# jackroos/VL-BERT

Hardware: AMD Instinct MI355X
Metric: samples/sec VL-BERT-base pretrain (seq 64+36 regions) at 1/2/4/8 MI355X (higher is better)
Workload: dtype bf16; 1 GPU; VL-BERT-base 12-layer pretrain step (fwd+bwd+clip+AdamW), 64 text + 36 regions, precomputed 2048-d region features, dropout on; global_batch=256, per_gpu_batch=256, per_gpu_caption_samples=256, per_gpu_text_only_samples=0, module=ResNetVLBERTForPretraining, seq_len=101, parallelism=dp1, hipgraph=False, arch=gfx950:sramecc+:xnack-, cus=256, forced_exchange=False, ranks=1

## Files before the change

vl-bert_amd/csrc/attention.hip:

```cpp
#include "vlb_common.h"

#define ATT_SP_MAX 256
#define ATT_D 64
#define ATT_THREADS 512

typedef __attribute__((ext_vector_type(4))) short s16x4;
typedef __attribute__((ext_vector_type(8))) short s16x8;

__device__ __forceinline__ int rho(int s) { return (s & ~31) | (((s >> 2) & 1) << 4) | (((s >> 3) & 3) << 2) | (s & 3); }
__device__ __forceinline__ int rm_addr(int row, int chunk) { return row * 128 + ((chunk ^ ((row >> 1) & 7)) << 4); }
__device__ __forceinline__ bf16x8 lds_frag(const char* base, int addr) { return *(const bf16x8*)(base + addr); }

__device__ __forceinline__ bf16x8 frag_perm(const char* img, int blk, int half, int c, int chunk) {
  return lds_frag(img, rm_addr(32 * blk + 16 * half + c, chunk));
}
__device__ __forceinline__ bf16x8 frag_nat(const char* img, int s0, int c, int chunk) {
  return lds_frag(img, rm_addr(rho(s0 + c), chunk));
}
__device__ __forceinline__ bf16x8 frag_tr(const char* img, int blk, int d0, int lane) {
  const int L = lane & 15, g = lane >> 4;
  const int b = d0 * 2 + (L & 3) * 8;
  const int r_lo = 32 * blk + 4 * g + (L >> 2);
  const int r_hi = r_lo + 16;
  const int a_lo = r_lo * 128 + ((((b >> 4) ^ ((r_lo >> 1) & 7)) << 4) | (b & 15));
  const int a_hi = r_hi * 128 + ((((b >> 4) ^ ((r_hi >> 1) & 7)) << 4) | (b & 15));
  const s16x4 lo = __builtin_amdgcn_ds_read_tr16_b64_v4i16((__attribute__((address_space(3))) s16x4*)(img + a_lo));
  const s16x4 hi = __builtin_amdgcn_ds_read_tr16_b64_v4i16((__attribute__((address_space(3))) s16x4*)(img + a_hi));
  const s16x8 v = __builtin_shufflevector(lo, hi, 0, 1, 2, 3, 4, 5, 6, 7);
  return __builtin_bit_cast(bf16x8, v);
}

template <int SP>
struct TileRegs {
  uint4 v[SP * 8 / ATT_THREADS];
};

template <int SP>
__device__ __forceinline__ void tile_load(const bf16_t* __restrict__ g, long ld, int S, int tid, TileRegs<SP>& r) {
#pragma unroll
  for (int it = 0; it < SP * 8 / ATT_THREADS; ++it) {
    const int P = it * ATT_THREADS + tid, s = min(P >> 3, S - 1), ch = P & 7;
    r.v[it] = *(const uint4*)(g + (long)s * ld + ch * 8);
  }
}

template <int SP>
__device__ __forceinline__ void tile_store(const TileRegs<SP>& r, int S, char* img, int tid) {
#pragma unroll
  for (int it = 0; it < SP * 8 / ATT_THREADS; ++it) {
    const int P = it * ATT_THREADS + tid, s = P >> 3, ch = P & 7;
    const bool in = s < S;
    const uint4 v = make_uint4(in ? r.v[it].x : 0u, in ? r.v[it].y : 0u, in ? r.v[it].z : 0u, in ? r.v[it].w : 0u);
    *(uint4*)(img + rm_addr(rho(s), ch)) = v;
  }
}

template <int SP>
__device__ __forceinline__ void rowdot_store(const TileRegs<SP>& a_, const TileRegs<SP>& o_, int S, float* sD, int tid) {
#pragma unroll
  for (int it = 0; it < SP * 8 / ATT_THREADS; ++it) {
    const int P = it * ATT_THREADS + tid, row = P >> 3, ch = P & 7;
    const uint4 a = a_.v[it], o = o_.v[it];
    float d = bflo(a.x) * bflo(o.x) + bfhi(a.x) * bfhi(o.x) + bflo(a.y) * bflo(o.y) + bfhi(a.y) * bfhi(o.y) +
              bflo(a.z) * bflo(o.z) + bfhi(a.z) * bfhi(o.z) + bflo(a.w) * bflo(o.w) + bfhi(a.w) * bfhi(o.w);
    d = row < S ? d : 0.f;
    d += __shfl_xor(d, 1, 64);
    d += __shfl_xor(d, 2, 64);
    d += __shfl_xor(d, 4, 64);
    if (ch == 0) sD[row] = d;
  }
}

__device__ __forceinline__ bf16x8 pack8(const float* v) {
  uint32_t w[4] = {pack2bf(v[0], v[1]), pack2bf(v[2], v[3]), pack2bf(v[4], v[5]), pack2bf(v[6], v[7])};
  return __builtin_bit_cast(bf16x8, *(uint4*)w);
}

__device__ __forceinline__ void drop8(float* v, uint32_t key, uint32_t base, uint32_t thr, float scale) {
  const uint32_t odd = base & 1u, p0 = base >> 1;
  uint32_t h[5];
#pragma unroll
  for (int k = 0; k < 5; ++k) h[k] = vlb_pair_hash(p0 + k, key);
#pragma unroll
  for (int k = 0; k < 4; ++k) {
    const uint32_t w = __builtin_amdgcn_alignbit(h[k + 1], h[k], odd << 4);
    v[2 * k] = ((w & 0xffffu) >= thr) ? v[2 * k] * scale : 0.f;
    v[2 * k + 1] = ((w >> 16) >= thr) ? v[2 * k + 1] * scale : 0.f;
  }
}

struct AttnParams {
  const bf16_t* qkv;
  const float* mask;
  bf16_t* ctx;
  float* lse;
  const bf16_t* dctx;
  bf16_t* dqkv;
  int B, S, H, nh;
  float scale;
  uint32_t drop_thr; float drop_scale; const uint32_t* seed; uint32_t tag;
};

template <int NU, int QS>
__global__ __launch_bounds__(ATT_THREADS, NU <= 4 ? 4 : 2) void attn_fwd_kernel(const AttnParams p) {
  constexpr int ATT_SP = 32 * NU, TILE_BYTES = ATT_SP * ATT_D * 2;
  extern __shared__ __attribute__((aligned(16))) char smem[];
  char* sK = smem;
  char* sV = smem + TILE_BYTES;
  float* sMB = (float*)(smem + 2 * TILE_BYTES);

  const int tid = threadIdx.x, lane = tid & 63, wave = tid >> 6;
  const int c = lane & 15, g = lane >> 4;
  const int b = blockIdx.x / p.nh, h = blockIdx.x % p.nh;
  const int S = p.S;
  const long ld = 3L * p.H;
  const bf16_t* qbase = p.qkv + (long)b * S * ld + h * ATT_D;
  TileRegs<ATT_SP> rk, rv;
  tile_load<ATT_SP>(qbase + p.H, ld, S, tid, rk);
  tile_load<ATT_SP>(qbase + 2 * p.H, ld, S, tid, rv);
  bf16x8 qf[2];
  auto load_q = [&](int q0) {
    const int q = min(q0 + c, S - 1);
#pragma unroll
    for (int ds = 0; ds < 2; ++ds) qf[ds] = *(const bf16x8*)(qbase + (long)q * ld + ds * 32 + g * 8);
  };
  load_q(wave * 16);
  const float mrow = p.mask[b * S + min(tid, S - 1)];
  const uint32_t seed = (p.drop_thr && p.seed) ? *p.seed : 0u;
  tile_store<ATT_SP>(rk, S, sK, tid);
  tile_store<ATT_SP>(rv, S, sV, tid);
  if (tid < ATT_SP) sMB[tid] = (tid < S) ? (1.0f - mrow) * -10000.0f : -INFINITY;
  __syncthreads();
  const uint32_t key = vlb_rng_key(seed, p.tag);
  const int U = (S + 31) >> 5;

#pragma unroll 1
  for (int qs = 0; qs < QS; ++qs) {
  const int q0 = (wave + 8 * qs) * 16;
  if (q0 >= S) break;
  if (qs > 0) load_q(q0);

  f32x4 sc[NU][2];
#pragma unroll
  for (int u = 0; u < NU; ++u)
#pragma unroll
    for (int hf = 0; hf < 2; ++hf) {
      sc[u][hf] = (f32x4){0.f, 0.f, 0.f, 0.f};
      if (u < U) {
#pragma unroll
        for (int ds = 0; ds < 2; ++ds)
          sc[u][hf] = VLB_MFMA_16x16x32(frag_perm(sK, u, hf, c, ds * 4 + g), qf[ds], sc[u][hf], 0, 0, 0);
      }
    }

  float mx = -INFINITY;
#pragma unroll
  for (int u = 0; u < NU; ++u)
#pragma unroll
    for (int hf = 0; hf < 2; ++hf)
#pragma unroll
      for (int r = 0; r < 4; ++r) {
        const float v = (u < U) ? sc[u][hf][r] * p.scale + sMB[32 * u + 8 * g + 4 * hf + r] : -INFINITY;
        sc[u][hf][r] = v;
        mx = fmaxf(mx, v);
      }
  mx = fmaxf(mx, __shfl_xor(mx, 16, 64));
  mx = fmaxf(mx, __shfl_xor(mx, 32, 64));
  float sum = 0.f;
#pragma unroll
  for (int u = 0; u < NU; ++u)
#pragma unroll
    for (int hf = 0; hf < 2; ++hf)
#pragma unroll
      for (int r = 0; r < 4; ++r) {
        const float e = __expf(sc[u][hf][r] - mx);
        sc[u][hf][r] = e;
        sum += e;
      }
  sum += __shfl_xor(sum, 16, 64);
  sum += __shfl_xor(sum, 32, 64);
  const float inv = 1.0f / sum;
  const int q = q0 + c;
  if (g == 0 && q < S) p.lse[((long)b * p.nh + h) * S + q] = mx + __logf(sum);

  const uint32_t qrow = ((uint32_t)(b * p.nh + h) * (uint32_t)S + (uint32_t)min(q, S - 1)) * (uint32_t)S;
  bf16x8 pf[NU];
#pragma unroll
  for (int u = 0; u < NU; ++u) {
    float v[8];
#pragma unroll
    for (int hf = 0; hf < 2; ++hf)
#pragma unroll
      for (int r = 0; r < 4; ++r) v[4 * hf + r] = sc[u][hf][r] * inv;
    if (p.drop_thr) drop8(v, key, qrow + 32u * u + 8u * g, p.drop_thr, p.drop_scale);
    pf[u] = pack8(v);
  }

  bf16_t* orow = p.ctx + ((long)b * S + min(q, S - 1)) * p.H + h * ATT_D + 4 * g;
#pragma unroll
  for (int dt = 0; dt < 4; ++dt) {
    f32x4 o = {0.f, 0.f, 0.f, 0.f};
#pragma unroll
    for (int u = 0; u < NU; ++u)
      if (u < U) o = VLB_MFMA_16x16x32(frag_tr(sV, u, dt * 16, lane), pf[u], o, 0, 0, 0);
    if (q < S) *(uint2*)(orow + dt * 16) = make_uint2(pack2bf(o[0], o[1]), pack2bf(o[2], o[3]));
  }
  }
}

template <int NU, int QS>
__global__ __launch_bounds__(ATT_THREADS, NU <= 4 ? 4 : 2) void attn_bwd_kernel(const AttnParams p) {
  constexpr int ATT_SP = 32 * NU, TILE_BYTES = ATT_SP * ATT_D * 2;
  extern __shared__ __attribute__((aligned(16))) char smem[];
  char* sQ = smem;
  char* sK = smem + 1 * TILE_BYTES;
  char* sV = smem + 2 * TILE_BYTES;
  char* sdO = smem + 3 * TILE_BYTES;
  float* sMB = (float*)(smem + 4 * TILE_BYTES);
  float* sLSE = sMB + ATT_SP;
  float* sD = sLSE + ATT_SP;

  const int tid = threadIdx.x, lane = tid & 63, wave = tid >> 6;
  const int c = lane & 15, g = lane >> 4;
  const int b = blockIdx.x / p.nh, h = blockIdx.x % p.nh;
  const int S = p.S;
  const long ld = 3L * p.H;
  const bf16_t* qbase = p.qkv + (long)b * S * ld + h * ATT_D;
  const bf16_t* dobase = p.dctx + (long)b * S * p.H + h * ATT_D;
  const bf16_t* obase = p.ctx + (long)b * S * p.H + h * ATT_D;
  TileRegs<ATT_SP> rq, rk, rv, rdo, ro;
  tile_load<ATT_SP>(qbase, ld, S, tid, rq);
  tile_load<ATT_SP>(qbase + p.H, ld, S, tid, rk);
  tile_load<ATT_SP>(qbase + 2 * p.H, ld, S, tid, rv);
  tile_load<ATT_SP>(dobase, p.H, S, tid, rdo);
  tile_load<ATT_SP>(obase, p.H, S, tid, ro);
  const float mrow = p.mask[b * S + min(tid, S - 1)];
  const float lrow = p.lse[((long)b * p.nh + h) * S + min(tid, S - 1)];
  const uint32_t seed = (p.drop_thr && p.seed) ? *p.seed : 0u;
  tile_store<ATT_SP>(rq, S, sQ, tid);
  tile_store<ATT_SP>(rk, S, sK, tid);
  tile_store<ATT_SP>(rv, S, sV, tid);
  tile_store<ATT_SP>(rdo, S, sdO, tid);
  rowdot_store<ATT_SP>(rdo, ro, S, sD, tid);
  if (tid < ATT_SP) {
    sMB[tid] = (tid < S) ? (1.0f - mrow) * -10000.0f : -INFINITY;
    sLSE[tid] = (tid < S) ? lrow : 0.f;
  }
  __syncthreads();

  const uint32_t key = vlb_rng_key(seed, p.tag);
  const uint32_t bh = (uint32_t)(b * p.nh + h);
  const int U = (S + 31) >> 5;
#pragma unroll 1
  for (int qs = 0; qs < QS; ++qs) {
  const int w16 = (wave + 8 * qs) * 16;
  if (w16 >= S) break;
  const int pos = w16 + c;
  const bool pos_ok = pos < S;

  {
    bf16x8 kf[2], vf[2];
#pragma unroll
    for (int ds = 0; ds < 2; ++ds) {
      kf[ds] = frag_nat(sK, w16, c, ds * 4 + g);
      vf[ds] = frag_nat(sV, w16, c, ds * 4 + g);
    }
    f32x4 dv[4], dk[4];
#pragma unroll
    for (int dt = 0; dt < 4; ++dt) dv[dt] = dk[dt] = (f32x4){0.f, 0.f, 0.f, 0.f};
    const float mb = sMB[pos];
    const uint32_t kcol = (uint32_t)min(pos, S - 1);
#pragma unroll (NU <= 4 ? NU : 1)
    for (int v = 0; v < NU; ++v) {
      if (v < U) {
        float pv[8], dsv[8];
#pragma unroll
        for (int hf = 0; hf < 2; ++hf) {
          f32x4 s = {0.f, 0.f, 0.f, 0.f}, dp = {0.f, 0.f, 0.f, 0.f};
#pragma unroll
          for (int ds = 0; ds < 2; ++ds) {
            s = VLB_MFMA_16x16x32(frag_perm(sQ, v, hf, c, ds * 4 + g), kf[ds], s, 0, 0, 0);
            dp = VLB_MFMA_16x16x32(frag_perm(sdO, v, hf, c, ds * 4 + g), vf[ds], dp, 0, 0, 0);
          }
#pragma unroll
          for (int r = 0; r < 4; ++r) {
            const int q = 32 * v + 8 * g + 4 * hf + r;
            const float pr = __expf(s[r] * p.scale + mb - sLSE[q]);
            float keepf = 1.f;
            if (p.drop_thr) {
              const uint32_t idx = (bh * (uint32_t)S + (uint32_t)min(q, S - 1)) * (uint32_t)S + kcol;
              const uint32_t hsh = vlb_pair_hash(idx >> 1, key);
              keepf = (((idx & 1u) ? (hsh >> 16) : (hsh & 0xffffu)) >= p.drop_thr) ? p.drop_scale : 0.f;
            }
            pv[4 * hf + r] = pr * keepf;
            dsv[4 * hf + r] = pr * (dp[r] * keepf - sD[q]);
          }
        }
        const bf16x8 pd = pack8(pv), dsf = pack8(dsv);
#pragma unroll
        for (int dt = 0; dt < 4; ++dt) {
          dv[dt] = VLB_MFMA_16x16x32(frag_tr(sdO, v, dt * 16, lane), pd, dv[dt], 0, 0, 0);
          dk[dt] = VLB_MFMA_16x16x32(frag_tr(sQ, v, dt * 16, lane), dsf, dk[dt], 0, 0, 0);
        }
      }
    }
    if (pos_ok) {
      bf16_t* orow = p.dqkv + ((long)b * S + pos) * ld + h * ATT_D + 4 * g;
#pragma unroll
      for (int dt = 0; dt < 4; ++dt) {
        *(uint2*)(orow + p.H + dt * 16) = make_uint2(pack2bf(dk[dt][0] * p.scale, dk[dt][1] * p.scale),
                                                     pack2bf(dk[dt][2] * p.scale, dk[dt][3] * p.scale));
        *(uint2*)(orow + 2 * p.H + dt * 16) = make_uint2(pack2bf(dv[dt][0], dv[dt][1]), pack2bf(dv[dt][2], dv[dt][3]));
      }
    }
  }

  {
    bf16x8 qf[2], dof[2];
#pragma unroll
    for (int ds = 0; ds < 2; ++ds) {
      qf[ds] = frag_nat(sQ, w16, c, ds * 4 + g);
      dof[ds] = frag_nat(sdO, w16, c, ds * 4 + g);
    }
    f32x4 dq[4];
#pragma unroll
    for (int dt = 0; dt < 4; ++dt) dq[dt] = (f32x4){0.f, 0.f, 0.f, 0.f};
    const float lse = sLSE[pos], dd = sD[pos];
    const uint32_t qrow = (bh * (uint32_t)S + (uint32_t)min(pos, S - 1)) * (uint32_t)S;
#pragma unroll (NU <= 4 ? NU : 1)
    for (int u = 0; u < NU; ++u) {
      if (u < U) {
        float pr[8], dpv[8];
#pragma unroll
        for (int hf = 0; hf < 2; ++hf) {
          f32x4 s = {0.f, 0.f, 0.f, 0.f}, dp = {0.f, 0.f, 0.f, 0.f};
#pragma unroll
          for (int ds = 0; ds < 2; ++ds) {
            s = VLB_MFMA_16x16x32(frag_perm(sK, u, hf, c, ds * 4 + g), qf[ds], s, 0, 0, 0);
            dp = VLB_MFMA_16x16x32(frag_perm(sV, u, hf, c, ds * 4 + g), dof[ds], dp, 0, 0, 0);
          }
#pragma unroll
          for (int r = 0; r < 4; ++r) {
            pr[4 * hf + r] = __expf(s[r] * p.scale + sMB[32 * u + 8 * g + 4 * hf + r] - lse);
            dpv[4 * hf + r] = dp[r];
          }
        }
        if (p.drop_thr) drop8(dpv, key, qrow + 32u * u + 8u * g, p.drop_thr, p.drop_scale);
        float dsv[8];
#pragma unroll
        for (int j = 0; j < 8; ++j) dsv[j] = pr[j] * (dpv[j] - dd);
        const bf16x8 dsf = pack8(dsv);
#pragma unroll
        for (int dt = 0; dt < 4; ++dt)
          dq[dt] = VLB_MFMA_16x16x32(frag_tr(sK, u, dt * 16, lane), dsf, dq[dt], 0, 0, 0);
      }
    }
    if (pos_ok) {
      bf16_t* orow = p.dqkv + ((long)b * S + pos) * ld + h * ATT_D + 4 * g;
#pragma unroll
      for (int dt = 0; dt < 4; ++dt)
        *(uint2*)(orow + dt * 16) = make_uint2(pack2bf(dq[dt][0] * p.scale, dq[dt][1] * p.scale),
                                               pack2bf(dq[dt][2] * p.scale, dq[dt][3] * p.scale));
    }
  }
  }
}

__device__ __forceinline__ int pt_addr(int row, int chunk16) { return row * 256 + ((chunk16 ^ (row & 15)) << 4); }

__device__ __forceinline__ bf16x8 frag_pt(const char* img, int v, int key0, int lane) {
  const int L = lane & 15, g = lane >> 4;
  const int r_lo = 32 * v + 8 * g + (L >> 2), r_hi = r_lo + 4;
  const int cb = key0 * 2 + (L & 3) * 8;
  const int a_lo = pt_addr(r_lo, cb >> 4) | (cb & 15), a_hi = pt_addr(r_hi, cb >> 4) | (cb & 15);
  const s16x4 lo = __builtin_amdgcn_ds_read_tr16_b64_v4i16((__attribute__((address_space(3))) s16x4*)(img + a_lo));
  const s16x4 hi = __builtin_amdgcn_ds_read_tr16_b64_v4i16((__attribute__((address_space(3))) s16x4*)(img + a_hi));
  const s16x8 w = __builtin_shufflevector(lo, hi, 0, 1, 2, 3, 4, 5, 6, 7);
  return __builtin_bit_cast(bf16x8, w);
}

__global__ __launch_bounds__(ATT_THREADS, 4) void attn_bwd2_kernel(const AttnParams p) {
  constexpr int NU = 4, ATT_SP = 128, TILE_BYTES = ATT_SP * ATT_D * 2;
  extern __shared__ __attribute__((aligned(16))) char smem[];
  char* sQ = smem;
  char* sK = smem + 1 * TILE_BYTES;
  char* sV = smem + 2 * TILE_BYTES;
  char* sdO = smem + 3 * TILE_BYTES;
  char* sT = sK;
  float* sMB = (float*)(smem + 4 * TILE_BYTES);
  float* sLSE = sMB + ATT_SP;
  float* sD = sLSE + ATT_SP;

  const int tid = threadIdx.x, lane = tid & 63, wave = tid >> 6;
  const int c = lane & 15, g = lane >> 4;
  const int b = blockIdx.x / p.nh, h = blockIdx.x % p.nh;
  const int S = p.S;
  const long ld = 3L * p.H;
  const bf16_t* qbase = p.qkv + (long)b * S * ld + h * ATT_D;
  const bf16_t* dobase = p.dctx + (long)b * S * p.H + h * ATT_D;
  const bf16_t* obase = p.ctx + (long)b * S * p.H + h * ATT_D;
  TileRegs<ATT_SP> rq, rk, rv, rdo, ro;
  tile_load<ATT_SP>(qbase, ld, S, tid, rq);
  tile_load<ATT_SP>(qbase + p.H, ld, S, tid, rk);
  tile_load<ATT_SP>(qbase + 2 * p.H, ld, S, tid, rv);
  tile_load<ATT_SP>(dobase, p.H, S, tid, rdo);
  tile_load<ATT_SP>(obase, p.H, S, tid, ro);
  const float mrow = p.mask[b * S + min(tid, S - 1)];
  const float lrow = p.lse[((long)b * p.nh + h) * S + min(tid, S - 1)];
  const uint32_t seed = (p.drop_thr && p.seed) ? *p.seed : 0u;
  tile_store<ATT_SP>(rq, S, sQ, tid);
  tile_store<ATT_SP>(rk, S, sK, tid);
  tile_store<ATT_SP>(rv, S, sV, tid);
  tile_store<ATT_SP>(rdo, S, sdO, tid);
  rowdot_store<ATT_SP>(rdo, ro, S, sD, tid);
  if (tid < ATT_SP) {
    sMB[tid] = (tid < S) ? (1.0f - mrow) * -10000.0f : -INFINITY;
    sLSE[tid] = (tid < S) ? lrow : 0.f;
  }
  __syncthreads();

  const uint32_t key = vlb_rng_key(seed, p.tag);
  const uint32_t bh = (uint32_t)(b * p.nh + h);
  const int U = (S + 31) >> 5;
  const int w16 = wave * 16;
  const int pos = w16 + c;
  const bool pos_ok = pos < S;
  const bool active = w16 < 32 * U;

  bf16x8 pd[NU], dsf[NU];
#pragma unroll
  for (int u = 0; u < NU; ++u) pd[u] = dsf[u] = (bf16x8){0, 0, 0, 0, 0, 0, 0, 0};
  if (w16 < S) {
    bf16x8 qf[2], dof[2];
#pragma unroll
    for (int ds = 0; ds < 2; ++ds) {
      qf[ds] = frag_nat(sQ, w16, c, ds * 4 + g);
      dof[ds] = frag_nat(sdO, w16, c, ds * 4 + g);
    }
    f32x4 dq[4];
#pragma unroll
    for (int dt = 0; dt < 4; ++dt) dq[dt] = (f32x4){0.f, 0.f, 0.f, 0.f};
    const float lse = sLSE[pos], dd = sD[pos];
    const float rowf = pos_ok ? 1.f : 0.f;
    const uint32_t qrow = (bh * (uint32_t)S + (uint32_t)min(pos, S - 1)) * (uint32_t)S;
#pragma unroll
    for (int u = 0; u < NU; ++u) {
      if (u < U) {
        float pr[8], dpv[8], kv[8];
#pragma unroll
        for (int hf = 0; hf < 2; ++hf) {
          f32x4 sc = {0.f, 0.f, 0.f, 0.f}, dp = {0.f, 0.f, 0.f, 0.f};
#pragma unroll
          for (int ds = 0; ds < 2; ++ds) {
            sc = VLB_MFMA_16x16x32(frag_perm(sK, u, hf, c, ds * 4 + g), qf[ds], sc, 0, 0, 0);
            dp = VLB_MFMA_16x16x32(frag_perm(sV, u, hf, c, ds * 4 + g), dof[ds], dp, 0, 0, 0);
          }
#pragma unroll
          for (int r = 0; r < 4; ++r) {
            pr[4 * hf + r] = __expf(sc[r] * p.scale + sMB[32 * u + 8 * g + 4 * hf + r] - lse) * rowf;
            dpv[4 * hf + r] = dp[r];
            kv[4 * hf + r] = 1.f;
          }
        }
        if (p.drop_thr) drop8(kv, key, qrow + 32u * u + 8u * g, p.drop_thr, p.drop_scale);
        float pdv[8], dsv[8];
#pragma unroll
        for (int j = 0; j < 8; ++j) {
          pdv[j] = pr[j] * kv[j];
          dsv[j] = pr[j] * (dpv[j] * kv[j] - dd);
        }
        pd[u] = pack8(pdv);
        dsf[u] = pack8(dsv);
#pragma unroll
        for (int dt = 0; dt < 4; ++dt)
          dq[dt] = VLB_MFMA_16x16x32(frag_tr(sK, u, dt * 16, lane), dsf[u], dq[dt], 0, 0, 0);
      }
    }
    if (pos_ok) {
      bf16_t* orow = p.dqkv + ((long)b * S + pos) * ld + h * ATT_D + 4 * g;
#pragma unroll
      for (int dt = 0; dt < 4; ++dt)
        *(uint2*)(orow + dt * 16) = make_uint2(pack2bf(dq[dt][0] * p.scale, dq[dt][1] * p.scale),
                                               pack2bf(dq[dt][2] * p.scale, dq[dt][3] * p.scale));
    }
  }
  __syncthreads();

  f32x4 dv[4], dk[4];
#pragma unroll
  for (int dt = 0; dt < 4; ++dt) dv[dt] = dk[dt] = (f32x4){0.f, 0.f, 0.f, 0.f};
  if (active) {
#pragma unroll
    for (int u = 0; u < NU; ++u)
      if (u < U) *(bf16x8*)(sT + pt_addr(w16 + c, 4 * u + g)) = pd[u];
  }
  __syncthreads();
  if (w16 < S) {
#pragma unroll
    for (int v = 0; v < NU; ++v) {
      if (v < U) {
        const bf16x8 pt = frag_pt(sT, v, w16, lane);
#pragma unroll
        for (int dt = 0; dt < 4; ++dt)
          dv[dt] = VLB_MFMA_16x16x32(frag_tr(sdO, v, dt * 16, lane), pt, dv[dt], 0, 0, 0);
      }
    }
  }
  __syncthreads();
  if (active) {
#pragma unroll
    for (int u = 0; u < NU; ++u)
      if (u < U) *(bf16x8*)(sT + pt_addr(w16 + c, 4 * u + g)) = dsf[u];
  }
  __syncthreads();
  if (w16 < S) {
#pragma unroll
    for (int v = 0; v < NU; ++v) {
      if (v < U) {
        const bf16x8 st = frag_pt(sT, v, w16, lane);
#pragma unroll
        for (int dt = 0; dt < 4; ++dt)
          dk[dt] = VLB_MFMA_16x16x32(frag_tr(sQ, v, dt * 16, lane), st, dk[dt], 0, 0, 0);
      }
    }
    if (pos_ok) {
      bf16_t* orow = p.dqkv + ((long)b * S + pos) * ld + h * ATT_D + 4 * g;
#pragma unroll
      for (int dt = 0; dt < 4; ++dt) {
        *(uint2*)(orow + p.H + dt * 16) = make_uint2(pack2bf(dk[dt][0] * p.scale, dk[dt][1] * p.scale),
                                                     pack2bf(dk[dt][2] * p.scale, dk[dt][3] * p.scale));
        *(uint2*)(orow + 2 * p.H + dt * 16) = make_uint2(pack2bf(dv[dt][0], dv[dt][1]), pack2bf(dv[dt][2], dv[dt][3]));
      }
    }
  }
}

static int check_attn(const char* name, int B, int S, int H, int nh) {
  VLB_CHECK_ARG(B > 0 && S > 0 && S <= ATT_SP_MAX, "%s: S=%d unsupported (1..%d)", name, S, ATT_SP_MAX);
  VLB_CHECK_ARG(nh > 0 && H == nh * ATT_D, "%s: head dim must be 64 (H=%d, heads=%d)", name, H, nh);
  VLB_CHECK_ARG((long)B * nh * S * S < (1L << 32), "%s: dropout index overflow", name);
  return VLB_OK;
}

extern "C" int vlb_attention_fwd(const void* qkv, const float* mask, void* ctx, float* lse, int B, int S, int H, int nh,
                                 float drop_p, const uint32_t* seed, uint32_t tag, hipStream_t stream) {
  int rc = check_attn("vlb_attention_fwd", B, S, H, nh);
  if (rc) return rc;
  VLB_CHECK_ARG(qkv && mask && ctx && lse, "vlb_attention_fwd: null argument");
  VLB_CHECK_ARG(!(drop_p > 0.f) || seed, "vlb_attention_fwd: dropout needs a device seed pointer");
  AttnParams p;
  p.qkv = (const bf16_t*)qkv; p.mask = mask; p.ctx = (bf16_t*)ctx; p.lse = lse; p.dctx = nullptr; p.dqkv = nullptr;
  p.B = B; p.S = S; p.H = H; p.nh = nh; p.scale = 0.125f;
  p.drop_thr = vlb_drop_thr(drop_p); p.drop_scale = vlb_drop_scale(p.drop_thr); p.seed = seed; p.tag = tag;
  if (S <= 128) {
    const int smem = 2 * (128 * ATT_D * 2) + 128 * 4;
    hipLaunchKernelGGL((attn_fwd_kernel<4, 1>), dim3(B * nh), dim3(ATT_THREADS), smem, stream, p);
  } else {
    const int smem = 2 * (256 * ATT_D * 2) + 256 * 4;
    static bool attr_set = false;
    if (!attr_set) {
      (void)hipFuncSetAttribute((const void*)attn_fwd_kernel<8, 2>, hipFuncAttributeMaxDynamicSharedMemorySize, smem);
      attr_set = true;
    }
    hipLaunchKernelGGL((attn_fwd_kernel<8, 2>), dim3(B * nh), dim3(ATT_THREADS), smem, stream, p);
  }
  VLB_CHECK_LAUNCH("vlb_attention_fwd");
  return VLB_OK;
}

extern "C" int vlb_attention_bwd(const void* qkv, const float* mask, const void* ctx, const float* lse, const void* dctx,
                                 void* dqkv, int B, int S, int H, int nh, float drop_p, const uint32_t* seed, uint32_t tag,
                                 hipStream_t stream) {
  int rc = check_attn("vlb_attention_bwd", B, S, H, nh);
  if (rc) return rc;
  VLB_CHECK_ARG(qkv && mask && ctx && lse && dctx && dqkv, "vlb_attention_bwd: null argument");
  VLB_CHECK_ARG(!(drop_p > 0.f) || seed, "vlb_attention_bwd: dropout needs a device seed pointer");
  AttnParams p;
  p.qkv = (const bf16_t*)qkv; p.mask = mask; p.ctx = (bf16_t*)ctx; p.lse = (float*)lse; p.dctx = (const bf16_t*)dctx;
  p.dqkv = (bf16_t*)dqkv;
  p.B = B; p.S = S; p.H = H; p.nh = nh; p.scale = 0.125f;
  p.drop_thr = vlb_drop_thr(drop_p); p.drop_scale = vlb_drop_scale(p.drop_thr); p.seed = seed; p.tag = tag;
  static bool attr_set = false;
  if (!attr_set) {
    (void)hipFuncSetAttribute((const void*)attn_bwd_kernel<4, 1>, hipFuncAttributeMaxDynamicSharedMemorySize, 4 * (128 * ATT_D * 2) + 3 * 128 * 4);
    (void)hipFuncSetAttribute((const void*)attn_bwd2_kernel, hipFuncAttributeMaxDynamicSharedMemorySize, 4 * (128 * ATT_D * 2) + 3 * 128 * 4);
    (void)hipFuncSetAttribute((const void*)attn_bwd_kernel<8, 2>, hipFuncAttributeMaxDynamicSharedMemorySize, 4 * (256 * ATT_D * 2) + 3 * 256 * 4);
    attr_set = true;
  }
  static int bwd2 = -1;
  if (bwd2 < 0) {
    const char* v = getenv("VLB_ATTN_BWD2");
    bwd2 = v ? atoi(v) : 1;
  }
  if (S <= 128 && bwd2)
    hipLaunchKernelGGL(attn_bwd2_kernel, dim3(B * nh), dim3(ATT_THREADS), 4 * (128 * ATT_D * 2) + 3 * 128 * 4, stream, p);
  else if (S <= 128)
    hipLaunchKernelGGL((attn_bwd_kernel<4, 1>), dim3(B * nh), dim3(ATT_THREADS), 4 * (128 * ATT_D * 2) + 3 * 128 * 4, stream, p);
  else
    hipLaunchKernelGGL((attn_bwd_kernel<8, 2>), dim3(B * nh), dim3(ATT_THREADS), 4 * (256 * ATT_D * 2) + 3 * 256 * 4, stream, p);
  VLB_CHECK_LAUNCH("vlb_attention_bwd");
  return VLB_OK;
}
```

Before: 13170 samples/s.

## Stage attention backward dQ/dK/dV through LDS for coalesced row stores

In attn_bwd2_kernel, the dQ, dK and dV outputs are written into a per-wave LDS staging area (reusing the dO tile region) and then flushed as full 16-byte row chunks. This replaces the scattered 8-byte strided global stores. The LDS swizzle keys for the row-major and transposed tiles are also changed, to cut bank conflicts on the read_tr and staging accesses. The change adds wave-level fences plus extra LDS traffic, and it depends on sdO no longer being read when the staging writes happen.

```diff
diff --git a/vl-bert_amd/csrc/attention.hip b/vl-bert_amd/csrc/attention.hip
--- a/vl-bert_amd/csrc/attention.hip
+++ b/vl-bert_amd/csrc/attention.hip
@@ -8,7 +8,8 @@
 typedef __attribute__((ext_vector_type(8))) short s16x8;
 
 __device__ __forceinline__ int rho(int s) { return (s & ~31) | (((s >> 2) & 1) << 4) | (((s >> 3) & 3) << 2) | (s & 3); }
-__device__ __forceinline__ int rm_addr(int row, int chunk) { return row * 128 + ((chunk ^ ((row >> 1) & 7)) << 4); }
+__device__ __forceinline__ int rm_key(int row) { return ((row >> 1) & 3) << 1; }
+__device__ __forceinline__ int rm_addr(int row, int chunk) { return row * 128 + ((chunk ^ rm_key(row)) << 4); }
 __device__ __forceinline__ bf16x8 lds_frag(const char* base, int addr) { return *(const bf16x8*)(base + addr); }
 
 __device__ __forceinline__ bf16x8 frag_perm(const char* img, int blk, int half, int c, int chunk) {
@@ -22,8 +23,8 @@
   const int b = d0 * 2 + (L & 3) * 8;
   const int r_lo = 32 * blk + 4 * g + (L >> 2);
   const int r_hi = r_lo + 16;
-  const int a_lo = r_lo * 128 + ((((b >> 4) ^ ((r_lo >> 1) & 7)) << 4) | (b & 15));
-  const int a_hi = r_hi * 128 + ((((b >> 4) ^ ((r_hi >> 1) & 7)) << 4) | (b & 15));
+  const int a_lo = rm_addr(r_lo, b >> 4) | (b & 15);
+  const int a_hi = rm_addr(r_hi, b >> 4) | (b & 15);
   const s16x4 lo = __builtin_amdgcn_ds_read_tr16_b64_v4i16((__attribute__((address_space(3))) s16x4*)(img + a_lo));
   const s16x4 hi = __builtin_amdgcn_ds_read_tr16_b64_v4i16((__attribute__((address_space(3))) s16x4*)(img + a_hi));
   const s16x8 v = __builtin_shufflevector(lo, hi, 0, 1, 2, 3, 4, 5, 6, 7);
@@ -74,6 +75,26 @@
 __device__ __forceinline__ bf16x8 pack8(const float* v) {
   uint32_t w[4] = {pack2bf(v[0], v[1]), pack2bf(v[2], v[3]), pack2bf(v[4], v[5]), pack2bf(v[6], v[7])};
   return __builtin_bit_cast(bf16x8, *(uint4*)w);
+}
+
+__device__ __forceinline__ int st_addr(int row, int chunk) { return row * 128 + ((chunk ^ (row & 7)) << 4); }
+__device__ __forceinline__ void wave_lds_sync() {
+  __builtin_amdgcn_fence(__ATOMIC_RELEASE, "wavefront");
+  __builtin_amdgcn_wave_barrier();
+  __builtin_amdgcn_fence(__ATOMIC_ACQUIRE, "wavefront");
+}
+__device__ __forceinline__ void stage_put(char* st, int c, int g, int dt, uint2 v) {
+  *(uint2*)(st + st_addr(c, 2 * dt + (g >> 1)) + (((g & 1) ^ (c >> 3)) << 3)) = v;
+}
+__device__ __forceinline__ void stage_flush(const char* st, bf16_t* __restrict__ out, long ld, int row0, int S, int lane) {
+  wave_lds_sync();
+#pragma unroll
+  for (int it = 0; it < 2; ++it) {
+    const int row = 8 * it + (lane >> 3), ch = lane & 7;
+    const uint4 v = *(const uint4*)(st + st_addr(row, ch));
+    if (row0 + row < S) *(uint4*)(out + (long)(row0 + row) * ld + ch * 8) = it ? make_uint4(v.z, v.w, v.x, v.y) : v;
+  }
+  wave_lds_sync();
 }
 
 __device__ __forceinline__ void drop8(float* v, uint32_t key, uint32_t base, uint32_t thr, float scale) {
@@ -366,7 +387,10 @@
   }
 }
 
-__device__ __forceinline__ int pt_addr(int row, int chunk16) { return row * 256 + ((chunk16 ^ (row & 15)) << 4); }
+__device__ __forceinline__ int pt_addr(int row, int chunk16) {
+  const int key = (((row >> 3) & 1) << 3) | ((row & 3) << 1) | ((row >> 2) & 1);
+  return row * 256 + ((chunk16 ^ key) << 4);
+}
 
 __device__ __forceinline__ bf16x8 frag_pt(const char* img, int v, int key0, int lane) {
   const int L = lane & 15, g = lane >> 4;
@@ -428,8 +452,11 @@
   const bool active = w16 < 32 * U;
 
   bf16x8 pd[NU], dsf[NU];
+  uint2 dqp[4];
 #pragma unroll
   for (int u = 0; u < NU; ++u) pd[u] = dsf[u] = (bf16x8){0, 0, 0, 0, 0, 0, 0, 0};
+#pragma unroll
+  for (int dt = 0; dt < 4; ++dt) dqp[dt] = make_uint2(0u, 0u);
   if (w16 < S) {
     bf16x8 qf[2], dof[2];
 #pragma unroll
@@ -476,13 +503,9 @@
           dq[dt] = VLB_MFMA_16x16x32(frag_tr(sK, u, dt * 16, lane), dsf[u], dq[dt], 0, 0, 0);
       }
     }
-    if (pos_ok) {
-      bf16_t* orow = p.dqkv + ((long)b * S + pos) * ld + h * ATT_D + 4 * g;
-#pragma unroll
-      for (int dt = 0; dt < 4; ++dt)
-        *(uint2*)(orow + dt * 16) = make_uint2(pack2bf(dq[dt][0] * p.scale, dq[dt][1] * p.scale),
-                                               pack2bf(dq[dt][2] * p.scale, dq[dt][3] * p.scale));
-    }
+#pragma unroll
+    for (int dt = 0; dt < 4; ++dt)
+      dqp[dt] = make_uint2(pack2bf(dq[dt][0] * p.scale, dq[dt][1] * p.scale), pack2bf(dq[dt][2] * p.scale, dq[dt][3] * p.scale));
   }
   __syncthreads();
 
@@ -512,6 +535,16 @@
     for (int u = 0; u < NU; ++u)
       if (u < U) *(bf16x8*)(sT + pt_addr(w16 + c, 4 * u + g)) = dsf[u];
   }
+  char* st = sdO + wave * 2048;
+  bf16_t* obh = p.dqkv + (long)b * S * ld + h * ATT_D;
+  if (w16 < S) {
+#pragma unroll
+    for (int dt = 0; dt < 4; ++dt) stage_put(st, c, g, dt, dqp[dt]);
+    stage_flush(st, obh, ld, w16, S, lane);
+#pragma unroll
+    for (int dt = 0; dt < 4; ++dt) stage_put(st, c, g, dt, make_uint2(pack2bf(dv[dt][0], dv[dt][1]), pack2bf(dv[dt][2], dv[dt][3])));
+    stage_flush(st, obh + 2 * p.H, ld, w16, S, lane);
+  }
   __syncthreads();
   if (w16 < S) {
 #pragma unroll
@@ -523,15 +556,11 @@
           dk[dt] = VLB_MFMA_16x16x32(frag_tr(sQ, v, dt * 16, lane), st, dk[dt], 0, 0, 0);
       }
     }
-    if (pos_ok) {
-      bf16_t* orow = p.dqkv + ((long)b * S + pos) * ld + h * ATT_D + 4 * g;
-#pragma unroll
-      for (int dt = 0; dt < 4; ++dt) {
-        *(uint2*)(orow + p.H + dt * 16) = make_uint2(pack2bf(dk[dt][0] * p.scale, dk[dt][1] * p.scale),
-                                                     pack2bf(dk[dt][2] * p.scale, dk[dt][3] * p.scale));
-        *(uint2*)(orow + 2 * p.H + dt * 16) = make_uint2(pack2bf(dv[dt][0], dv[dt][1]), pack2bf(dv[dt][2], dv[dt][3]));
-      }
-    }
+#pragma unroll
+    for (int dt = 0; dt < 4; ++dt)
+      stage_put(st, c, g, dt, make_uint2(pack2bf(dk[dt][0] * p.scale, dk[dt][1] * p.scale),
+                                         pack2bf(dk[dt][2] * p.scale, dk[dt][3] * p.scale)));
+    stage_flush(st, obh + p.H, ld, w16, S, lane);
   }
 }
 
```

After: 13260 samples/s (median of 6 runs). About the same (+0.7%).
